# gnosisguild/pvw-rs

Measured on AMD Instinct MI355X. Metric: parties/s for n-party encrypt (pvw::crypto::encrypt); achieved HBM GB/s vs peak, higher is better.
Workload: dtype u64

## Files before the change

pvw_rs_amd/csrc/pvw_capi.hip:

```cpp
#include <hip/hip_runtime.h>

#include <algorithm>
#include <atomic>
#include <chrono>
#include <cmath>
#include <cstdio>
#include <cstring>
#include <functional>
#include <map>
#include <mutex>
#include <string>
#include <thread>
#include <vector>

#include "../../include/pvw_hip.h"
#include "pvw_arith.h"
#include "pvw_bignum.h"
#include "pvw_chacha.h"
#include "pvw_decode.h"
#include "pvw_kernels.h"
#include "pvw_shamir_fields.h"
#if PVW_TUNING
#include "../../include/pvw_hip_tuning.h"
#endif
// ... 107 lines not shown
  u64* gtmpB = nullptr;
  u64* gtmpK = nullptr;
  u64* shares = nullptr;
  size_t shares_bytes = 0;
  u64* interp = nullptr;
  size_t interp_bytes = 0;
  u64* interp_wide = nullptr;
  size_t interp_wide_bytes = 0;
  u64* packw = nullptr;
  size_t packw_bytes = 0;
  u64* packw_wide = nullptr;
  size_t packw_wide_bytes = 0;
  u64* handover_wide = nullptr;
  size_t handover_wide_bytes = 0;
  u64* handover_io = nullptr;
  size_t handover_io_bytes = 0;
  u64* correct = nullptr;
  size_t correct_bytes = 0;
  u64* correct_wide = nullptr;
  size_t correct_wide_bytes = 0;
  hipStream_t aux = nullptr;
  bool aux_used = false;
  std::vector<hipEvent_t> events;
  AheadRing ahead;
  char* ahead_block = nullptr;
  size_t ahead_set_bytes = 0, ahead_rhat_bytes = 0;
  std::vector<hipEvent_t> ahead_done;
  hipEvent_t ahead_guard[2] = {nullptr, nullptr};
  hipEvent_t ahead_mark = nullptr;
  hipEvent_t ahead_last = nullptr;
  bool ahead_off = false;
  struct Span { void* p; size_t bytes; bool cleared; };
  std::vector<Span> secrets, wiped;
  size_t rhat_public_from = SIZE_MAX;
};
static void ws_mark_secret(Workspace* w, void* p, size_t bytes, bool cleared = false) {
  if (!p || !bytes) return;
  if (p == (void*)w->rhat && w->rhat_public_from < bytes) w->rhat_public_from = bytes;
  for (Workspace::Span& sp : w->secrets)
    if (sp.p == p) { sp.bytes = bytes > sp.bytes ? bytes : sp.bytes; sp.cleared = cleared; return; }
  w->secrets.push_back(Workspace::Span{p, bytes, cleared});
}
static void ws_public(Workspace* w, void* p, size_t bytes) {
  if (!p || !bytes) return;
  const char *lo = (const char*)p, *hi = lo + bytes;
  for (const Workspace::Span& sp : w->secrets)
// ... 403 lines not shown
  hipFree(w->gtmpA);
  hipFree(w->gtmpB);
  hipFree(w->gtmpK);
  if (w->shares) hipMemset(w->shares, 0, w->shares_bytes);
  hipFree(w->shares);
  hipFree(w->interp);
  hipFree(w->interp_wide);
  hipFree(w->packw);
  hipFree(w->packw_wide);
  hipFree(w->handover_wide);
  if (w->handover_io) hipMemset(w->handover_io, 0, w->handover_io_bytes);
  hipFree(w->handover_io);
  if (w->correct) hipMemset(w->correct, 0, w->correct_bytes);
  hipFree(w->correct);
  if (w->correct_wide) hipMemset(w->correct_wide, 0, w->correct_wide_bytes);
  hipFree(w->correct_wide);
  for (hipEvent_t e : w->events) hipEventDestroy(e);
  if (w->ahead_block) hipMemset(w->ahead_block, 0, w->ahead_set_bytes * w->ahead.slots());
  hipFree(w->ahead_block);
  for (hipEvent_t e : w->ahead_done) hipEventDestroy(e);
  for (hipEvent_t e : w->ahead_guard) if (e) hipEventDestroy(e);
  if (w->ahead_mark) hipEventDestroy(w->ahead_mark);
  if (w->aux) hipStreamDestroy(w->aux);
  if (w->own_stream && w->stream) hipStreamDestroy(w->stream);
  delete w;
}
static int32_t ws_acquire(pvw_ctx* c, Workspace** out) {
  {
    std::lock_guard<std::mutex> g(c->mu);
    if (!c->pool.empty()) {
      *out = c->pool.back();
      c->pool.pop_back();
      return PVW_OK;
    }
  }
  Workspace* w = new Workspace();
  if (hipStreamCreateWithFlags(&w->stream, hipStreamNonBlocking) != hipSuccess) {
    delete w;
    return fail(PVW_ERR_INTERNAL, "hipStreamCreate failed");
  }
  w->own_stream = true;
  int32_t rc = ws_alloc(c, w);
  if (rc != PVW_OK) { ws_free(w); return rc; }
  *out = w;
  return PVW_OK;
}
// ... 115 lines not shown
  DealerKeys piece(size_t i) const { return by_state ? *this : from(i); }
  template <class Batch>
  void fill(Batch& b, u32 count) const {
    if (by_state) {
      b.rnd = st->dev;
      b.rnd_off = first;
    } else {
      for (u32 x = 0; x < count; ++x) b.key[x] = make_key(seeds + (first + x) * 32);
    }
  }
};

static int32_t ws_aux(Workspace* w, size_t events) {
  if (!w->aux) PVW_HIP(hipStreamCreateWithFlags(&w->aux, hipStreamNonBlocking));
  while (w->events.size() < events) {
    hipEvent_t e;
    PVW_HIP(hipEventCreateWithFlags(&e, hipEventDisableTiming));
    w->events.push_back(e);
  }
  w->aux_used = true;
  return PVW_OK;
}

template <class Body>
static int32_t host_call(pvw_ctx* c, Body&& body) {
  Workspace* w;
  PVW_TRY(ws_acquire(c, &w));
  int32_t rc = body(w);
  auto keep = [&](hipError_t e, const char* what) {
    if (e != hipSuccess && rc == PVW_OK) rc = fail(PVW_ERR_INTERNAL, std::string(what) + " failed: " + hipGetErrorString(e));
  };
  if (w->aux_used) keep(hipStreamSynchronize(w->aux), "helper stream sync");
  w->aux_used = false;
  keep(ws_wipe_secrets(w, w->stream), "wipe");
  keep(hipStreamSynchronize(w->stream), "stream sync");
  ws_release(c, w);
  return rc;
}

static bool multi_uses_gemm(size_t D) {
  const int gemm_min = (int)PVW_ENV_INT("PVW_GEMM_MIN_DEALERS", 3);
  return gemm_min > 0 && D >= (size_t)gemm_min;
}
static int32_t multi_capture_check(pvw_ctx* c, hipStream_t s, size_t D) {
  if (!multi_uses_gemm(D) || !stream_capturing(s)) return PVW_OK;
  bool ready;
  {
    std::lock_guard<std::mutex> g(c->init_mu);
    ready = c->xm_valid;
  }
  {
    std::lock_guard<std::mutex> g(c->mu);
    auto it = c->async_ws.find((void*)s);
    const Workspace* w = it == c->async_ws.end() ? nullptr : it->second;
    ready = ready && w && w->vhat16 && w->yd && w->sy && (w->gtmpA || !c->rowsA()) && (w->gtmpB || !c->rowsB());
  }
// ... 6 lines not shown
static int32_t deal_capture_check(pvw_ctx* c, hipStream_t s, size_t D) {
  if (!stream_capturing(s)) return PVW_OK;
  bool ready;
  {
    std::lock_guard<std::mutex> g(c->mu);
    auto it = c->async_ws.find((void*)s);
    ready = it != c->async_ws.end() && it->second->shares;
  }
  if (!ready)
    return fail(PVW_ERR_INVALID_PARAMETERS, "multi-dealer encrypt under stream capture: call pvw_prepare(PVW_PREPARE_MFMA) on "
                                            "this stream first (and again after the matrices change)");
  return multi_capture_check(c, s, D);
}

static hipStream_t call_stream(const pvw_ctx* c, void* stream) { return stream ? (hipStream_t)stream : c->stream; }
static int32_t sum_prepare(pvw_ctx* c, Workspace* w, hipStream_t s);
static int32_t device_ws(pvw_ctx* c, void* stream, hipStream_t* s, Workspace** w) {
  *s = call_stream(c, stream);
  return ws_for_stream(c, *s, w);
}
static int32_t device_end(Workspace* w, hipStream_t s, int32_t rc) {
  if (rc != PVW_OK) {
    if (w->aux) (void)hipStreamSynchronize(w->aux);
    (void)hipStreamSynchronize(s);
  }
  if (ws_wipe_secrets(w, s) != hipSuccess && rc == PVW_OK) rc = fail(PVW_ERR_INTERNAL, "wipe failed");
  return rc;
}

template <class Pre, class Body>
static int32_t device_call(pvw_ctx* c, void* stream, Pre&& pre, Body&& body) {
  PVW_TRY(ensure_device(c));
  const hipStream_t s = call_stream(c, stream);
  PVW_TRY(pre(s));
  Workspace* w;
  PVW_TRY(ws_for_stream(c, s, &w));
  return device_end(w, s, body(w, s));
}
template <class Body>
static int32_t device_call(pvw_ctx* c, void* stream, Body&& body) {
  return device_call(c, stream, [](hipStream_t) { return (int32_t)PVW_OK; }, body);
}

static int32_t validate_params(const pvw_params_t* p) {
  if (!p) return fail(PVW_ERR_INVALID_PARAMETERS, "params is NULL");
  if (p->n == 0) return fail(PVW_ERR_INVALID_PARAMETERS, "n must be > 0");
// ... 2457 lines not shown
        ProfScope ps(c, "vec_digits", s);
        PVW_HIP(launch_vec_digits(vh, (size_t)k * P, w->yd, w->sy, nv, k, L, l, c->dt, s, 0, 0, c->xm_bytes));
      }
      ProfScope ps(c, "gemm_digits", s);
      GemmSection a{c->xmA, c1g, c1g, w->gtmpA, rA, 0, 0}, b{c->xmB, c2g, c2g, w->gtmpB, rB, 0, 0};
      std::vector<GemmErrSource> es;
      if (fused_e2) {
        for (u32 v0 = 0; v0 < nv; v0 += PVW_MAX_PROLOGUE_KEYS) {
          GemmErrSource e{};
          e.span = (nv - v0) < PVW_MAX_PROLOGUE_KEYS ? (nv - v0) : PVW_MAX_PROLOGUE_KEYS;
          keys.from(d0 + v0).fill(e, e.span);
          e.key_v = 1;
          e.domain = DOM_E2; e.index0 = c->party_lo; e.index_row = 1; e.index_v = 0; e.bound = c->b2;
          e.scalars = gsc + c->party_lo; e.scalar_v = c->n;
          es.push_back(e);
        }
        b.addend = nullptr;
      }
      if (rs && last) {
        GemmSection& fin = rB ? b : a;
        fin.rnd_ctr = &rs->counter;
        fin.rnd_adv = D;
      }
      PVW_HIP(launch_gemm_digits(a, b, w->yd, w->sy, c->dt, k, L, l, nv, (size_t)rA * P, (size_t)rB * P, s, nullptr, fused_e2 ? es.data() : nullptr, c->xm_bytes));
    } else {
      ProfScope ps(c, "mac_rows_multi", s);
      MacSection a(c->dA, c1g, c1g, rA), b(c->dB, c2g, c2g, rB);
      MultiVec mv{vh, (size_t)k * P, (size_t)rA * P, (size_t)rB * P, nv};
      if (rs && last) {
        a.rnd_ctr = &rs->counter;
        a.rnd_adv = D;
      }
      PVW_HIP(launch_mac_rows_multi(a, b, mv, c->dt, k, L, l, s));
    }
  }
  if (out_repr == PVW_REPR_POWER) {
    ProfScope ps(c, "intt", s);
    PVW_HIP(launch_ntt(d_c1, D * rA, true, c->dt, L, l, s));
    PVW_HIP(launch_ntt(d_c2, D * rB, true, c->dt, L, l, s));
  }
  return PVW_OK;
}

static int32_t encrypt_multi_checks(pvw_ctx* c, size_t D, size_t per_dealer, uint32_t out_repr) {
  PVW_TRY(check_repr(out_repr));
  if (D == 0) return fail(PVW_ERR_INVALID_PARAMETERS, "no dealers");
  if (per_dealer != c->n) {
// ... 3572 lines not shown
    PVW_TRY(cbd_job(c->variance, sj));
    draw.key = make_key(ks.sk_seed); draw.cbd_half = sj.cbd_half; draw.cbd_v = sj.cbd_v;
  } else {
    PVW_TRY(ws_aux(w, 2 * (size_t)nchunks + 2));
  }
  auto upload = [&](u32 ci, hipStream_t st) -> int32_t {
    const u32 q0 = a + ci * chunk, cn = (b - q0) < chunk ? (b - q0) : chunk;
    const size_t wd = (size_t)cn * k * l;
    i64* dst = d_small2[ci & 1];
    PVW_HIP(hipMemcpyAsync(dst, sk + (size_t)(q0 - lo) * k * l, wd * 8, hipMemcpyHostToDevice, st));
    if (ek) PVW_HIP(hipMemcpyAsync(dst + (size_t)chunk * k * l, ek + (size_t)(q0 - lo) * k * l, wd * 8, hipMemcpyHostToDevice, st));
    return PVW_OK;
  };
  if (!ks.seeded()) PVW_TRY(upload(0, s));
  PVW_HIP(launch_untile(c->dA, d_api, k, 0, k, L, l, false, c->dt, s));
  PVW_HIP(launch_vec_digits(d_api, P, d_yd, d_sy, k, k, L, l, c->dt, s, l, (size_t)k * P));
  for (u32 ci = 0; ci < nchunks; ++ci) {
    const u32 p0 = a + ci * chunk;
    const u32 cnt = (b - p0) < chunk ? (b - p0) : chunk;
    i64* d_small = d_small2[ci & 1];
    if (ci > 0 && !ks.seeded()) PVW_HIP(hipStreamWaitEvent(s, w->events[2 * ci], 0));
    ProfScope ps(c, "keygen", s);
    GemmSection ga{d_xm, d_erow, d_erow, d_tmp, cnt, 0, 0}, gb{nullptr, nullptr, nullptr, nullptr, 0, 0, 0};
    ga.tiled_out = c->dB;
    ga.tiled_row0 = p0 - c->party_lo;
    ga.tiled_swap = 1;
    ga.row_stride = (size_t)k * P;
    if (direct) {
      draw.party0 = p0;
      PVW_HIP(launch_shat_mftile(ks.seeded() ? nullptr : d_small, ks.seeded() ? &draw : nullptr, d_xm, cnt, k, L, l, c->dt, s));
      GemmErrSource es{};
      if (ek) { es.explicit_coeffs = d_small + (size_t)chunk * k * l; es.coef_row = k; es.coef_v = 1; }
      else es.key[0] = make_key(seed);
      es.domain = DOM_EKEY; es.index0 = p0 * k; es.index_row = k; es.index_v = 1; es.bound = c->b1;
      ga.addend = nullptr;
      ga.out = nullptr;
      PVW_HIP(launch_gemm_digits(ga, gb, d_yd, d_sy, c->dt, k, L, l, k, P, 0, s, &es));
    } else {
      PrologueBatch pb{};
      if (seed) pb.key[0] = make_key(seed);
      PrologueJob& js = pb.job[0];
      PrologueJob& je = pb.job[1];
      PVW_TRY(ks.job(c, pb, js, d_small, p0));
      js.out = d_srow; js.stride_poly = P; js.stride_limb = l; js.rep_out = (size_t)k * P;
      je.sj.kind = SAMPLE_UNIFORM; je.sj.domain = DOM_EKEY; je.sj.index0 = p0 * k; je.sj.count = k; je.sj.bound = c->b1;
      je.rep_index0 = k;
      if (ek) { je.explicit_coeffs = d_small + (size_t)chunk * k * l; je.rep_coeffs = (size_t)k * l; }
      je.out = d_erow; je.stride_poly = P; je.stride_limb = l; je.rep_out = (size_t)k * P;
      pb.njobs = 2;
      pb.reps = cnt;
      PVW_HIP(launch_prologue(pb, c->dt, L, l, s));
      PVW_HIP(hipMemsetAsync(d_xm, 0, xm_words(cnt, k, L, l) * 8, s));
      PVW_HIP(launch_mftile(d_srow, false, d_xm, cnt, k, L, l, s));
      PVW_HIP(launch_gemm_digits(ga, gb, d_yd, d_sy, c->dt, k, L, l, k, P, 0, s));
    }
    if (ks.seeded()) continue;
    PVW_HIP(hipEventRecord(w->events[2 * ci + 1], s));
    if (ci + 1 < nchunks) {
      if (ci >= 1) PVW_HIP(hipStreamWaitEvent(w->aux, w->events[2 * (ci - 1) + 1], 0));
      PVW_TRY(upload(ci + 1, w->aux));
      PVW_HIP(hipEventRecord(w->events[2 * ci + 2], w->aux));
    }
  }
  return PVW_OK;
}

static int32_t keygen_transposed(pvw_ctx* c, Workspace* w, u32 a, u32 b, u32 lo, const KeySource& ks, const int64_t* ek,
                                 const uint8_t* seed, bool use_gemm) {
  const u32 k = c->k, l = c->l, L = c->L;
  const size_t P = c->poly();
  hipStream_t s = w->stream;
  const u32 group = use_gemm ? 16 : 4;
  u32 sg = group;
  if (use_gemm) {
    const size_t per16 = yd_bytes(16, k, L, l);
    size_t m = ((size_t)2 << 30) / (per16 ? per16 : 1);
    if (m < 1) m = 1;
// ... 527 lines not shown
```

pvw_rs_amd/csrc/pvw_gemm.hip:

```cpp
#include <hip/hip_runtime.h>

#include "pvw_arith.h"
#include "pvw_chacha.h"
#include "pvw_decode.h"
#include "pvw_kernels.h"
#include "pvw_dev.h"

namespace pvw {

__global__ __launch_bounds__(64) void mfma_i8_probe_kernel(const signed char* __restrict__ A,
                                                            const signed char* __restrict__ B, int* __restrict__ Cm) {
  const u32 l = threadIdx.x, r = l & 31, h = l >> 5;
  union { v4i32 v; signed char b[16]; } fa, fb;
#pragma unroll
  for (int j = 0; j < 16; ++j) {
    fa.b[j] = A[r * 32 + 16 * h + j];
    fb.b[j] = B[(16 * h + j) * 32 + r];
  }
  v16i32 acc = {};
  acc = __builtin_amdgcn_mfma_i32_32x32x32_i8(fa.v, fb.v, acc, 0, 0, 0);
#pragma unroll
  for (int g = 0; g < 16; ++g) Cm[((g & 3) + 8 * (g >> 2) + 4 * h) * 32 + r] = acc[g];
}

// ... 661 lines not shown
  for (int r = 0; r < 2; ++r) {
    const u32 rt = rtbase + 2 * wr + r;
    if (rt >= RT || rt * 32 >= sec.nrows) continue;
    const u32 row = rt * 32 + rr;
#pragma unroll
    for (int g = 0; g < 4; ++g) {
      u64 res[2];
      if (biased) gemm_recombine_biased<FASTQ>(acc[r][g], m, inv32, res);
      else gemm_recombine<FASTQ>(acc[r][g], m, inv32, res);
#pragma unroll
      for (int pr = 0; pr < 2; ++pr) {
        const u32 v = g * 4 + pr + 2 * h;
        if (row < sec.nrows && v < nv)
          sec.tmp[vb * sec.tmp_bstride + (((size_t)limb * ELL + slot) * nv_pad + v) * rows_pad + row] = res[pr];
      }
    }
  }
}

#define PVW_FINISH_VPB (ELL >= 64 ? 2 : 4)
template <int ELL>
__global__ __launch_bounds__(256) void gemm_finish_kernel(GemmSection sec, const Mod* __restrict__ mods, u32 L,
                                                           u32 nv, u32 nv_pad, u32 rows_pad, size_t ostride,
                                                           const int* __restrict__ SY, size_t sy_b16) {
  constexpr int VPB = PVW_FINISH_VPB, PT = 32 * ELL / 256 ? 32 * ELL / 256 : 1;
  static_assert(sizeof(u64) * VPB * ELL * 33 <= 48 * 1024 || ELL > 32, "finish tiles");
  __shared__ u64 tile[VPB][ELL][33];
  rnd_advance(sec.rnd_ctr, sec.rnd_adv);
  const u32 rb = blockIdx.x, v0 = blockIdx.y * VPB, limb = blockIdx.z;
  const u32 row0 = rb * 32;
  u64 in[VPB][PT];
#pragma unroll
  for (int vi = 0; vi < VPB; ++vi) {
    const u32 v = (v0 + vi) < nv ? (v0 + vi) : (nv - 1);
    const u64* tp = sec.tmp + (v >> 4) * sec.tmp_bstride + (((size_t)limb * ELL) * nv_pad + (nv_pad == 16 ? (v & 15) : v)) * rows_pad + row0;
#pragma unroll
    for (int x = 0; x < PT; ++x) {
      const u32 e = threadIdx.x + 256 * x;
      const u32 row = e & 31, slot = (e >> 5) % ELL;
      in[vi][x] = tp[(size_t)slot * nv_pad * rows_pad + row];
    }
  }
#pragma unroll
  for (int vi = 0; vi < VPB; ++vi)
#pragma unroll
    for (int x = 0; x < PT; ++x) {
      const u32 e = threadIdx.x + 256 * x;
      if (e < 32 * ELL) tile[vi][(e >> 5) % ELL][e & 31] = in[vi][x];
    }
  __syncthreads();
  const u64 q = mods[limb].q;
  u64 add[VPB][PT];
// ... 18 lines not shown
#pragma unroll
    for (int x = 0; x < PT; ++x) {
      const u32 e = threadIdx.x + 256 * x;
      const u32 slot = e % ELL, row = e / ELL;
      if (e < 32 * ELL && row0 + row < sec.nrows && v0 + vi < nv) {
        const u64 val = addmod(tile[vi][slot][row], add[vi][x], q);
        if (sec.tiled_out) {
          constexpr u32 R = 128 / ELL;
          const u32 prow = sec.tiled_row0 + (sec.tiled_swap ? row0 + row : v0 + vi);
          const u32 pcol = sec.tiled_swap ? v0 + vi : row0 + row;
          const u32 ncol = sec.tiled_swap ? nv : sec.nrows;
          sec.tiled_out[(((size_t)(prow / R) * L + limb) * ncol + pcol) * 128 + (prow % R) * ELL + slot] = val;
        } else {
          const size_t o = (size_t)(v0 + vi) * ostride + (size_t)(row0 + row) * rstride + (size_t)limb * ELL + slot;
          sec.out[o] = val;
        }
      }
    }
}

template <int ELL, int VPB>
__global__ __launch_bounds__(32 * VPB) void gemm_finish_err_kernel(GemmSection sec, DevTables t, u32 L, u32 nv, u32 nv_pad, u32 rows_pad,
                                                               size_t ostride, const int* __restrict__ SY, size_t sy_b16, GemmErrSource es,
                                                               u32 v_lo, u32 v_hi) {
  constexpr int G = ELL / 2;
  constexpr int CST = ELL + 2;
  __shared__ i64 coef[32 * VPB * CST];
  const u32 tid = threadIdx.x, lane = tid & 63;
  const u32 row_raw = blockIdx.x * 32 + (tid & 31), v_raw = v_lo + blockIdx.y * VPB + (tid >> 5);
  const bool v_ok = v_raw < v_hi;
  const u32 row = row_raw < sec.nrows ? row_raw : sec.nrows - 1, v = v_ok ? v_raw : v_hi - 1;
  rnd_advance(sec.rnd_ctr, sec.rnd_adv);
  i64 c[ELL];
  __shared__ ChaChaKey vkey[VPB];
  if (es.rnd && !es.explicit_coeffs) {
    if ((tid & 31) == 0) vkey[tid >> 5] = call_seed(es.rnd->seed, es.rnd->base + es.rnd_off + (u64)(v - v_lo) * es.key_v);
    __builtin_amdgcn_fence(__ATOMIC_RELEASE, "wavefront");
    __builtin_amdgcn_wave_barrier();
    __builtin_amdgcn_fence(__ATOMIC_ACQUIRE, "wavefront");
  }
  {
    i64* o = coef + tid * CST;
    if (es.explicit_coeffs) {
      const i64* ec = es.explicit_coeffs + ((size_t)row * es.coef_row + (size_t)v * es.coef_v) * ELL;
#pragma unroll
      for (int sl = 0; sl < ELL; sl += 2) *reinterpret_cast<v2u64*>(o + sl) = *reinterpret_cast<const v2u64*>(ec + sl);
    } else {
      ChaChaRng g;
      g.init(es.rnd ? vkey[tid >> 5] : es.key[(v - v_lo) * es.key_v], es.domain, es.index0 + row * es.index_row + v * es.index_v);
      auto emit = [o](u32 sl, i64 val) { o[sl] = val; };
      sample_uniform_poly(g, ELL, es.bound, emit);
    }
#pragma unroll
    for (int sl = 0; sl < ELL; ++sl) c[sl] = o[sl];
  }
  const i64 scalar = es.scalars ? (i64)es.scalars[(size_t)v * es.scalar_v + row] : 0;
  const u64* tbase = sec.tmp + (v >> 4) * sec.tmp_bstride + (size_t)(nv_pad == 16 ? (v & 15) : v) * rows_pad + row;
  const size_t sstride = (size_t)nv_pad * rows_pad;
  const u64* cbase = reinterpret_cast<const u64*>(SY + (size_t)(v >> 4) * sy_b16 + ((size_t)((v & 15) >> 2) * L * ELL) * 32) + (v & 3);
  constexpr u32 R = 128 / ELL;
  const size_t rstride = sec.row_stride ? sec.row_stride : (size_t)L * ELL;
  u64 in[ELL];
  auto load_tmp = [&](u32 limb) {
#pragma unroll
    for (int sl = 0; sl < ELL; ++sl) in[sl] = __builtin_nontemporal_load(tbase + ((size_t)limb * ELL + sl) * sstride);
  };
  const u32 per = (L + gridDim.z - 1) / gridDim.z, limb_end = (blockIdx.z + 1) * per < L ? (blockIdx.z + 1) * per : L;
  u32 limb = blockIdx.z * per;
  if (limb < limb_end) load_tmp(limb);
  u64* stg = reinterpret_cast<u64*>(coef) + (size_t)(tid - lane) * CST;
  const u32 gi = lane & (G - 1), gb = lane & ~(u32)(G - 1);
  for (; limb < limb_end; ++limb) {
    const Mod m = t.mods[limb];
    u64 a[ELL], x[ELL];
#pragma unroll
    for (int sl = 0; sl < ELL; ++sl) { a[sl] = signed_residue(c[sl], m); x[sl] = in[sl]; }
    if (limb + 1 < limb_end) load_tmp(limb + 1);
    ntt_forward<ELL>(a, t.tw + (size_t)limb * ELL, t.twp + (size_t)limb * ELL, m);
    if (es.scalars) {
      const u64 mr = signed_residue(scalar, m);
      const u64* g = t.ghat + (size_t)limb * ELL;
      const u64* gp = t.ghatp + (size_t)limb * ELL;
#pragma unroll
      for (int sl = 0; sl < ELL; ++sl) a[sl] = addmod(a[sl], mulmod_shoup(mr, g[sl], gp[sl], m.q), m.q);
    }
#pragma unroll
    for (int sl = 0; sl < ELL; sl += 2) {
      const u64 c0 = cbase[((size_t)limb * ELL + sl) * 16], c1 = cbase[((size_t)limb * ELL + sl + 1) * 16];
      *reinterpret_cast<v2u64*>(stg + lane * CST + sl) =
          (v2u64){addmod(addmod(x[sl], a[sl], m.q), c0, m.q), addmod(addmod(x[sl + 1], a[sl + 1], m.q), c1, m.q)};
    }
// ... 71 lines not shown
  if (nv % 4) {
    const u32 NVG = (nv + 3) / 4, JB = gemm_ktiles(k, bytes);
    hipError_t e = hipMemsetAsync(YD + (size_t)(NVG - 1) * L * ell * JB * 1024, 0, (size_t)L * ell * JB * 1024, s);
    if (e != hipSuccess) return e;
    e = hipMemsetAsync(SY + (size_t)(NVG - 1) * L * ell * 32, 0, (size_t)L * ell * 32 * sizeof(int), s);
    if (e != hipSuccess) return e;
  }
  if (bytes == 7) {
    PVW_DISPATCH_ELL(ell, vec_digits7_kernel<E><<<dim3(nv * L * ell), dim3(64), 0, s>>>(vhat, vstride, YD, SY, nv, k, L, t, lstride, jstride));
    return hipGetLastError();
  }
#if PVW_TUNING
  static const int stage = (int)PVW_ENV_INT("PVW_VEC_DIGITS_STAGE", 1);
  if (!stage) {
    PVW_DISPATCH_ELL(ell, vec_digits_kernel<E, false><<<dim3(nv * L * ell), dim3(64), 0, s>>>(vhat, vstride, YD, SY, nv, k, L, t, lstride, jstride));
    return hipGetLastError();
  }
#endif
  PVW_DISPATCH_ELL(ell, vec_digits_kernel<E, true><<<dim3(nv * L * ell), dim3(64), 0, s>>>(vhat, vstride, YD, SY, nv, k, L, t, lstride, jstride));
  return hipGetLastError();
}

hipError_t launch_gemm_digits_core(GemmSection& sa, GemmSection& sb, const signed char* YD, const int* SY,
                                   const DevTables& t, u32 k, u32 L, u32 ell, u32 nv, hipStream_t s, u32 bytes) {
  const u32 kt = gemm_ktiles(k, bytes);
  sa.rt_groups = (sa.nrows + PVW_GEMM_ROWS_PER_WG - 1) / PVW_GEMM_ROWS_PER_WG;
  sb.rt_groups = (sb.nrows + PVW_GEMM_ROWS_PER_WG - 1) / PVW_GEMM_ROWS_PER_WG;
  const u32 blocks = (sa.rt_groups + sb.rt_groups) * L * ell;
  if (blocks == 0 || nv == 0) return hipSuccess;
  const u32 vbn = (nv + 15) / 16;
  const u32 NVG = vbn > 1 ? 4 : (nv + 3) / 4;
  const u32 nv_pad = NVG * 4;
  sa.tmp_bstride = (size_t)L * ell * 16 * sa.rt_groups * PVW_GEMM_ROWS_PER_WG;
  sb.tmp_bstride = (size_t)L * ell * 16 * sb.rt_groups * PVW_GEMM_ROWS_PER_WG;
  const size_t yd_b16 = (size_t)4 * L * ell * kt * 1024, sy_b16 = sy_bytes(16, L, ell) / sizeof(int);
#define PVW_GEMM_LAUNCH(G, N)                                                                                              \
  do {                                                                                                                    \
    if (t.min_q_bits >= 55) { PVW_DISPATCH_ELL(ell, gemm_digits_kernel<E, G, PVW_GEMM_RPW, N, true><<<dim3(blocks * vbn), dim3(256), 0, s>>>(sa, sb, YD, SY, t.mods, k, L, nv, nv_pad, vbn, yd_b16, sy_b16, kt)); } \
    else { PVW_DISPATCH_ELL(ell, gemm_digits_kernel<E, G, PVW_GEMM_RPW, N, false><<<dim3(blocks * vbn), dim3(256), 0, s>>>(sa, sb, YD, SY, t.mods, k, L, nv, nv_pad, vbn, yd_b16, sy_b16, kt)); } \
  } while (0)
#if PVW_TUNING
  if (PVW_ENV_INT("PVW_GEMM_ZERO_OPERANDS", 0)) {
    if (sa.nrows) (void)hipMemsetAsync(const_cast<u64*>(sa.XM), 0, xm_words(sa.nrows, k, L, ell) * 8, s);
    if (sb.nrows) (void)hipMemsetAsync(const_cast<u64*>(sb.XM), 0, xm_words(sb.nrows, k, L, ell) * 8, s);
    (void)hipMemsetAsync(const_cast<signed char*>(YD), 0, yd_b16 * vbn, s);
  }
#endif
  const bool wide = vbn >= 2 && k % 16 == 0 && k >= 16 && kt % 2 == 0 && PVW_ENV_INT("PVW_GEMM_WIDE", 1) != 0;
  if (wide) {
    const u32 ga = (sa.rt_groups * 4 + 7) / 8, gb2 = (sb.rt_groups * 4 + 7) / 8;
    const u32 wblocks = (ga + gb2) * L * ell * ((vbn + 1) / 2);
    if (t.min_q_bits >= 55) { PVW_DISPATCH_ELL(ell, gemm_digits_wide_kernel<E, true><<<dim3(wblocks), dim3(512), 0, s>>>(sa, sb, YD, t.mods, k, L, nv, nv_pad, vbn, yd_b16, kt)); }
    else { PVW_DISPATCH_ELL(ell, gemm_digits_wide_kernel<E, false><<<dim3(wblocks), dim3(512), 0, s>>>(sa, sb, YD, t.mods, k, L, nv, nv_pad, vbn, yd_b16, kt)); }
  } else {
  static const int unroll_ok = (int)PVW_ENV_INT("PVW_GEMM_UNROLL", 1);
  if (NVG == 4 && unroll_ok && kt == 64) { PVW_GEMM_LAUNCH(4, 8); }
  else if (NVG == 4 && unroll_ok && kt == 128) { PVW_GEMM_LAUNCH(4, 16); }
  else switch (NVG) {
    case 1: PVW_GEMM_LAUNCH(1, 0); break;
    case 2: PVW_GEMM_LAUNCH(2, 0); break;
    case 3: PVW_GEMM_LAUNCH(3, 0); break;
    case 4: PVW_GEMM_LAUNCH(4, 0); break;
    default: return hipErrorInvalidValue;
  }
#undef PVW_GEMM_LAUNCH
  }
  return hipGetLastError();
}

hipError_t launch_gemm_digits(const GemmSection& a, const GemmSection& b, const signed char* YD, const int* SY,
                              const DevTables& t, u32 k, u32 L, u32 ell, u32 nv, size_t ostride_a, size_t ostride_b,
                              hipStream_t s, const GemmErrSource* es_a, const GemmErrSource* es_b, u32 bytes) {
  GemmSection sa = a, sb = b;
  if ((sa.nrows == 0 && sb.nrows == 0) || nv == 0) return hipSuccess;
  {
    const hipError_t ge = launch_gemm_digits_core(sa, sb, YD, SY, t, k, L, ell, nv, s, bytes);
    if (ge != hipSuccess) return ge;
  }
  const u32 vbn = (nv + 15) / 16;
  const u32 nv_pad = (vbn > 1 ? 4 : (nv + 3) / 4) * 4;
  const size_t sy_b16 = sy_bytes(16, L, ell) / sizeof(int);
  auto finish = [&](const GemmSection& sec, size_t ostride, const GemmErrSource* es) -> hipError_t {
    if (!sec.nrows) return hipSuccess;
    const u32 rows_pad = sec.rt_groups * PVW_GEMM_ROWS_PER_WG;
    if (es) {
      if (ell > 32 || (sec.tiled_out && !sec.tiled_swap) || (!sec.tiled_out && !sec.out)) return hipErrorInvalidValue;
      for (u32 v_lo = 0; v_lo < nv; ++es) {
        const u32 span = es->span && es->span < nv - v_lo ? es->span : nv - v_lo, v_hi = v_lo + span;
        GemmSection sec_l = sec;
        if (v_hi < nv) sec_l.rnd_ctr = nullptr;
        const u32 gx = (sec.nrows + 31) / 32;
        bool one_wave = false;
#if PVW_TUNING
        one_wave = PVW_ENV_INT("PVW_FINISH_VPB", 8) == 2;
        if (one_wave) {
          const dim3 grid(gx, (span + 1) / 2, 1);
          switch (ell) {
            case 8: gemm_finish_err_kernel<8, 2><<<grid, dim3(64), 0, s>>>(sec_l, t, L, nv, nv_pad, rows_pad, ostride, SY, sy_b16, *es, v_lo, v_hi); break;
            case 16: gemm_finish_err_kernel<16, 2><<<grid, dim3(64), 0, s>>>(sec_l, t, L, nv, nv_pad, rows_pad, ostride, SY, sy_b16, *es, v_lo, v_hi); break;
            default: gemm_finish_err_kernel<32, 2><<<grid, dim3(64), 0, s>>>(sec_l, t, L, nv, nv_pad, rows_pad, ostride, SY, sy_b16, *es, v_lo, v_hi); break;
          }
        }
#endif
        if (!one_wave) {
          const u32 gy = (span + 7) / 8;
          u32 lz = 1;
          const size_t want = (size_t)PVW_ENV_INT("PVW_FINISH_BLOCKS", 4096);
          while (lz < L && (size_t)gx * gy * lz < want) lz *= 2;
          if (lz > L) lz = L;
          const dim3 grid(gx, gy, lz);
          switch (ell) {
            case 8: gemm_finish_err_kernel<8, 8><<<grid, dim3(256), 0, s>>>(sec_l, t, L, nv, nv_pad, rows_pad, ostride, SY, sy_b16, *es, v_lo, v_hi); break;
            case 16: gemm_finish_err_kernel<16, 8><<<grid, dim3(256), 0, s>>>(sec_l, t, L, nv, nv_pad, rows_pad, ostride, SY, sy_b16, *es, v_lo, v_hi); break;
            default: gemm_finish_err_kernel<32, 8><<<grid, dim3(256), 0, s>>>(sec_l, t, L, nv, nv_pad, rows_pad, ostride, SY, sy_b16, *es, v_lo, v_hi); break;
          }
        }
        v_lo = v_hi;
      }
      return hipGetLastError();
    }
    PVW_DISPATCH_ELL(ell, gemm_finish_kernel<E><<<dim3((sec.nrows + 31) / 32, (nv + (E >= 64 ? 2 : 4) - 1) / (E >= 64 ? 2 : 4), L), dim3(256), 0, s>>>(
                              sec, t.mods, L, nv, nv_pad, rows_pad, ostride, SY, sy_b16));
    return hipGetLastError();
  };
  hipError_t fe = finish(sa, ostride_a, es_a);
  if (fe != hipSuccess) return fe;
  return finish(sb, ostride_b, es_b);
}
static inline u32 ilog2_u32(u32 x) { u32 b = 0; while ((1u << b) < x) ++b; return b; }

__global__ __launch_bounds__(256) void gemm_finish_decrypt_kernel(const u64* __restrict__ tmp, size_t tmp_bstride, u32 nv_pad,
                                                                  u32 rows_pad, const int* __restrict__ SY, size_t sy_b16,
                                                                  const Mod* __restrict__ mods, u32 ell_log2, u32 P, u32 nrows,
                                                                  u32 nv, const u64* __restrict__ c2, size_t c2_vstride,
                                                                  size_t c2_rstride, u64* __restrict__ noisy) {
  constexpr u32 TR = 128, TF = 32;
  __shared__ __attribute__((aligned(16))) u64 tile[TR][TF + 2];
  const u32 r0 = blockIdx.x * TR, f0 = blockIdx.y * TF, v = blockIdx.z;
  const u32 wave = threadIdx.x >> 6, lane = threadIdx.x & 63;
  const u64* tb = tmp + (size_t)(v >> 4) * tmp_bstride + (size_t)(v & 15) * rows_pad + r0 + 2 * lane;
  const size_t fstride = (size_t)nv_pad * rows_pad;
  const u64* cb = reinterpret_cast<const u64*>(SY + (size_t)(v >> 4) * sy_b16 + (size_t)((v & 15) >> 2) * P * 32) + (v & 3);
  v2u64 x[TF / 4];
#pragma unroll
  for (u32 i = 0; i < TF / 4; ++i) {
    const u32 f = f0 + wave + 4 * i;
    if (f < P) x[i] = __builtin_nontemporal_load(reinterpret_cast<const v2u64*>(tb + (size_t)f * fstride));
  }
#pragma unroll
  for (u32 i = 0; i < TF / 4; ++i) {
// ... 58 lines not shown
```

pvw_rs_amd/csrc/pvw_kernels.h:

```cpp
#pragma once
#include <hip/hip_runtime.h>

#include "pvw_arith.h"
#include "pvw_chacha.h"
#include "pvw_decode.h"
#include "pvw_wide.h"

#ifndef PVW_TUNING
#define PVW_TUNING 0
#endif
#if PVW_TUNING
#include <cstdlib>
#define PVW_ENV_INT(name, dflt) ([]() -> long { const char* e_ = getenv(name); return e_ ? atol(e_) : (long)(dflt); }())
#else
#define PVW_ENV_INT(name, dflt) ((long)(dflt))
#endif

namespace pvw {

enum { DOM_R = 0, DOM_E1 = 1, DOM_E2 = 2, DOM_SK = 3, DOM_EKEY = 4, DOM_CRS = 5, DOM_GAUSS = 6, DOM_PK = 7, DOM_CALL = 8 };

struct RndState {
  u32 seed[8];
  u64 counter;
// ... 427 lines not shown
                         const Mod* mods = nullptr);
struct ShatDraw {
  ChaChaKey key;
  u32 cbd_half, cbd_v;
  u32 party0;
};
hipError_t launch_shat_mftile(const i64* coeffs, const ShatDraw* draw, u64* XM, u32 rows, u32 k, u32 L, u32 ell, const DevTables& t,
                              hipStream_t s);
hipError_t launch_vec_digits(const u64* vhat, size_t vstride, signed char* YD, int* SY, u32 nv, u32 k, u32 L, u32 ell,
                             const DevTables& t, hipStream_t s, size_t lstride = 0, size_t jstride = 0, u32 bytes = 8);
struct GemmErrSource {
  u32 span;
  const i64* explicit_coeffs;
  size_t coef_row, coef_v;
  ChaChaKey key[PVW_MAX_PROLOGUE_KEYS];
  u32 key_v;
  u32 domain, index0, index_row, index_v;
  u64 bound;
  const u64* scalars;
  size_t scalar_v;
  const RndState* rnd;
  u64 rnd_off;
};
hipError_t launch_gemm_digits(const GemmSection& a, const GemmSection& b, const signed char* YD, const int* SY,
                              const DevTables& t, u32 k, u32 L, u32 ell, u32 nv, size_t ostride_a, size_t ostride_b,
                              hipStream_t s, const GemmErrSource* es_a = nullptr, const GemmErrSource* es_b = nullptr, u32 bytes = 8);
hipError_t launch_gemm_digits_core(GemmSection& a, GemmSection& b, const signed char* YD, const int* SY, const DevTables& t, u32 k,
                                   u32 L, u32 ell, u32 nv, hipStream_t s, u32 bytes = 8);
hipError_t launch_finish_decrypt(const GemmSection& a, const int* SY, const DevTables& t, u32 L, u32 ell, u32 nv, const u64* c2,
                                 size_t c2_vstride, size_t c2_rstride, u64* noisy, hipStream_t s);
hipError_t launch_reduce_words(const u64* src, u64* dst, size_t words, const DevTables& t, u32 L, u32 ell, hipStream_t s);
#if PVW_TUNING
hipError_t read_stamps(u64* out, u32* hw, u32 count);
hipError_t init_probe_attributes();
hipError_t launch_read_probe(const u64* M, size_t total_tiles, u32 tiles_per_wave, u64* sink, hipStream_t s);
hipError_t launch_read_probe2(const u64* M, size_t total_tiles, u32 tiles_per_wave, u64* sink, u32 U, bool dbuf, u32 lds_bytes,
                              hipStream_t s, u32 xmap = 0);
#endif
hipError_t init_kernel_attributes();
hipError_t launch_mfma_probe(const signed char* A, const signed char* B, int* C, hipStream_t s);
hipError_t launch_decode(u64* noisy, u64* out, size_t count, const DecodeTables& t, hipStream_t s, const DevTables* xf = nullptr,
                         u64* wipe = nullptr, size_t wipe_bytes = 0, bool* wiped = nullptr, u64* noise = nullptr,
                         u32* status = nullptr, const PlainArgs* plain = nullptr);

hipError_t launch_wire_pack(const u64* words, size_t count, unsigned char* out, const Mod* mods, u32 L, u32 ell, hipStream_t s);
hipError_t launch_wire_unpack(const unsigned char* in, size_t count, u64* words, unsigned long long* bad, const Mod* mods, u32 L,
                              u32 ell, hipStream_t s);
hipError_t init_wire_attributes();

}
```

Baseline: 22.47 million.

## Split GEMM by limb ranges and overlap finish kernels on a side stream

Partitions the multi-dealer GEMM and its finish step into limb ranges (two by default). Each range's GEMM runs on the main stream while the previous range's finish or error-injection kernel runs on a dedicated side stream, joined by events. The goal is to hide finish-kernel time behind GEMM work. The cost is extra launches, event traffic and a second stream, and it is disabled under stream capture.

```diff
diff --git a/pvw_rs_amd/csrc/pvw_capi.hip b/pvw_rs_amd/csrc/pvw_capi.hip
--- a/pvw_rs_amd/csrc/pvw_capi.hip
+++ b/pvw_rs_amd/csrc/pvw_capi.hip
@@ -153,6 +153,10 @@
   hipStream_t aux = nullptr;
   bool aux_used = false;
   std::vector<hipEvent_t> events;
+  hipStream_t fin = nullptr;
+  bool fin_used = false;
+  bool fin_off = false;
+  hipEvent_t fin_ev[GemmRanges::MAX + 1] = {};
   AheadRing ahead;
   char* ahead_block = nullptr;
   size_t ahead_set_bytes = 0, ahead_rhat_bytes = 0;
@@ -602,6 +606,8 @@
   for (hipEvent_t e : w->ahead_guard) if (e) hipEventDestroy(e);
   if (w->ahead_mark) hipEventDestroy(w->ahead_mark);
   if (w->aux) hipStreamDestroy(w->aux);
+  for (hipEvent_t e : w->fin_ev) if (e) hipEventDestroy(e);
+  if (w->fin) hipStreamDestroy(w->fin);
   if (w->own_stream && w->stream) hipStreamDestroy(w->stream);
   delete w;
 }
@@ -763,6 +769,32 @@
   return PVW_OK;
 }
 
+#define PVW_GEMM_FINISH_RANGES_ENCRYPT 2
+#define PVW_GEMM_FINISH_RANGES_KEYGEN 2
+static const GemmRanges* ws_gemm_ranges(Workspace* w, hipStream_t s, u32 measured, GemmRanges& gr) {
+  long z = PVW_ENV_INT("PVW_GEMM_FINISH_RANGES", 0);
+  if (z <= 0) z = measured;
+  if (z > GemmRanges::MAX) z = GemmRanges::MAX;
+  if (z <= 1 || w->fin_off || stream_capturing(s)) return nullptr;
+  if (!w->fin) {
+    bool ok = hipStreamCreateWithFlags(&w->fin, hipStreamNonBlocking) == hipSuccess;
+    for (hipEvent_t& e : w->fin_ev) ok = ok && hipEventCreateWithFlags(&e, hipEventDisableTiming) == hipSuccess;
+    if (!ok) {
+      (void)hipGetLastError();
+      for (hipEvent_t& e : w->fin_ev) { if (e) hipEventDestroy(e); e = nullptr; }
+      if (w->fin) hipStreamDestroy(w->fin);
+      w->fin = nullptr;
+      w->fin_off = true;
+      return nullptr;
+    }
+  }
+  w->fin_used = true;
+  gr.side = w->fin;
+  gr.ev = w->fin_ev;
+  gr.ranges = (u32)z;
+  return &gr;
+}
+
 template <class Body>
 static int32_t host_call(pvw_ctx* c, Body&& body) {
   Workspace* w;
@@ -773,6 +805,8 @@
   };
   if (w->aux_used) keep(hipStreamSynchronize(w->aux), "helper stream sync");
   w->aux_used = false;
+  if (w->fin_used) keep(hipStreamSynchronize(w->fin), "finish stream sync");
+  w->fin_used = false;
   keep(ws_wipe_secrets(w, w->stream), "wipe");
   keep(hipStreamSynchronize(w->stream), "stream sync");
   ws_release(c, w);
@@ -825,6 +859,7 @@
 static int32_t device_end(Workspace* w, hipStream_t s, int32_t rc) {
   if (rc != PVW_OK) {
     if (w->aux) (void)hipStreamSynchronize(w->aux);
+    if (w->fin) (void)hipStreamSynchronize(w->fin);
     (void)hipStreamSynchronize(s);
   }
   if (ws_wipe_secrets(w, s) != hipSuccess && rc == PVW_OK) rc = fail(PVW_ERR_INTERNAL, "wipe failed");
@@ -3328,7 +3363,9 @@
         fin.rnd_ctr = &rs->counter;
         fin.rnd_adv = D;
       }
-      PVW_HIP(launch_gemm_digits(a, b, w->yd, w->sy, c->dt, k, L, l, nv, (size_t)rA * P, (size_t)rB * P, s, nullptr, fused_e2 ? es.data() : nullptr, c->xm_bytes));
+      GemmRanges gr;
+      PVW_HIP(launch_gemm_digits(a, b, w->yd, w->sy, c->dt, k, L, l, nv, (size_t)rA * P, (size_t)rB * P, s, nullptr, fused_e2 ? es.data() : nullptr, c->xm_bytes,
+                                 ws_gemm_ranges(w, s, PVW_GEMM_FINISH_RANGES_ENCRYPT, gr)));
     } else {
       ProfScope ps(c, "mac_rows_multi", s);
       MacSection a(c->dA, c1g, c1g, rA), b(c->dB, c2g, c2g, rB);
@@ -6947,6 +6984,7 @@
     if (ci > 0 && !ks.seeded()) PVW_HIP(hipStreamWaitEvent(s, w->events[2 * ci], 0));
     ProfScope ps(c, "keygen", s);
     GemmSection ga{d_xm, d_erow, d_erow, d_tmp, cnt, 0, 0}, gb{nullptr, nullptr, nullptr, nullptr, 0, 0, 0};
+    GemmRanges gr;
     ga.tiled_out = c->dB;
     ga.tiled_row0 = p0 - c->party_lo;
     ga.tiled_swap = 1;
@@ -6960,7 +6998,7 @@
       es.domain = DOM_EKEY; es.index0 = p0 * k; es.index_row = k; es.index_v = 1; es.bound = c->b1;
       ga.addend = nullptr;
       ga.out = nullptr;
-      PVW_HIP(launch_gemm_digits(ga, gb, d_yd, d_sy, c->dt, k, L, l, k, P, 0, s, &es));
+      PVW_HIP(launch_gemm_digits(ga, gb, d_yd, d_sy, c->dt, k, L, l, k, P, 0, s, &es, nullptr, 8, ws_gemm_ranges(w, s, PVW_GEMM_FINISH_RANGES_KEYGEN, gr)));
     } else {
       PrologueBatch pb{};
       if (seed) pb.key[0] = make_key(seed);
@@ -6977,7 +7015,7 @@
       PVW_HIP(launch_prologue(pb, c->dt, L, l, s));
       PVW_HIP(hipMemsetAsync(d_xm, 0, xm_words(cnt, k, L, l) * 8, s));
       PVW_HIP(launch_mftile(d_srow, false, d_xm, cnt, k, L, l, s));
-      PVW_HIP(launch_gemm_digits(ga, gb, d_yd, d_sy, c->dt, k, L, l, k, P, 0, s));
+      PVW_HIP(launch_gemm_digits(ga, gb, d_yd, d_sy, c->dt, k, L, l, k, P, 0, s, nullptr, nullptr, 8, ws_gemm_ranges(w, s, PVW_GEMM_FINISH_RANGES_KEYGEN, gr)));
     }
     if (ks.seeded()) continue;
     PVW_HIP(hipEventRecord(w->events[2 * ci + 1], s));
diff --git a/pvw_rs_amd/csrc/pvw_gemm.hip b/pvw_rs_amd/csrc/pvw_gemm.hip
--- a/pvw_rs_amd/csrc/pvw_gemm.hip
+++ b/pvw_rs_amd/csrc/pvw_gemm.hip
@@ -707,12 +707,12 @@
 template <int ELL>
 __global__ __launch_bounds__(256) void gemm_finish_kernel(GemmSection sec, const Mod* __restrict__ mods, u32 L,
                                                            u32 nv, u32 nv_pad, u32 rows_pad, size_t ostride,
-                                                           const int* __restrict__ SY, size_t sy_b16) {
+                                                           const int* __restrict__ SY, size_t sy_b16, u32 limb0) {
   constexpr int VPB = PVW_FINISH_VPB, PT = 32 * ELL / 256 ? 32 * ELL / 256 : 1;
   static_assert(sizeof(u64) * VPB * ELL * 33 <= 48 * 1024 || ELL > 32, "finish tiles");
   __shared__ u64 tile[VPB][ELL][33];
   rnd_advance(sec.rnd_ctr, sec.rnd_adv);
-  const u32 rb = blockIdx.x, v0 = blockIdx.y * VPB, limb = blockIdx.z;
+  const u32 rb = blockIdx.x, v0 = blockIdx.y * VPB, limb = limb0 + blockIdx.z;
   const u32 row0 = rb * 32;
   u64 in[VPB][PT];
 #pragma unroll
@@ -777,7 +777,7 @@
 template <int ELL, int VPB>
 __global__ __launch_bounds__(32 * VPB) void gemm_finish_err_kernel(GemmSection sec, DevTables t, u32 L, u32 nv, u32 nv_pad, u32 rows_pad,
                                                                size_t ostride, const int* __restrict__ SY, size_t sy_b16, GemmErrSource es,
-                                                               u32 v_lo, u32 v_hi) {
+                                                               u32 v_lo, u32 v_hi, u32 limb0, u32 nl) {
   constexpr int G = ELL / 2;
   constexpr int CST = ELL + 2;
   __shared__ i64 coef[32 * VPB * CST];
@@ -820,8 +820,8 @@
 #pragma unroll
     for (int sl = 0; sl < ELL; ++sl) in[sl] = __builtin_nontemporal_load(tbase + ((size_t)limb * ELL + sl) * sstride);
   };
-  const u32 per = (L + gridDim.z - 1) / gridDim.z, limb_end = (blockIdx.z + 1) * per < L ? (blockIdx.z + 1) * per : L;
-  u32 limb = blockIdx.z * per;
+  const u32 per = (nl + gridDim.z - 1) / gridDim.z, limb_end = limb0 + ((blockIdx.z + 1) * per < nl ? (blockIdx.z + 1) * per : nl);
+  u32 limb = limb0 + blockIdx.z * per;
   if (limb < limb_end) load_tmp(limb);
   u64* stg = reinterpret_cast<u64*>(coef) + (size_t)(tid - lane) * CST;
   const u32 gi = lane & (G - 1), gb = lane & ~(u32)(G - 1);
@@ -939,11 +939,14 @@
 }
 
 hipError_t launch_gemm_digits_core(GemmSection& sa, GemmSection& sb, const signed char* YD, const int* SY,
-                                   const DevTables& t, u32 k, u32 L, u32 ell, u32 nv, hipStream_t s, u32 bytes) {
+                                   const DevTables& t, u32 k, u32 L, u32 ell, u32 nv, hipStream_t s, u32 bytes, u32 limb0,
+                                   u32 nl) {
   const u32 kt = gemm_ktiles(k, bytes);
   sa.rt_groups = (sa.nrows + PVW_GEMM_ROWS_PER_WG - 1) / PVW_GEMM_ROWS_PER_WG;
   sb.rt_groups = (sb.nrows + PVW_GEMM_ROWS_PER_WG - 1) / PVW_GEMM_ROWS_PER_WG;
-  const u32 blocks = (sa.rt_groups + sb.rt_groups) * L * ell;
+  if (nl == 0) { limb0 = 0; nl = L; }
+  if (limb0 + nl > L) return hipErrorInvalidValue;
+  const u32 blocks = (sa.rt_groups + sb.rt_groups) * nl * ell;
   if (blocks == 0 || nv == 0) return hipSuccess;
   const u32 vbn = (nv + 15) / 16;
   const u32 NVG = vbn > 1 ? 4 : (nv + 3) / 4;
@@ -951,10 +954,19 @@
   sa.tmp_bstride = (size_t)L * ell * 16 * sa.rt_groups * PVW_GEMM_ROWS_PER_WG;
   sb.tmp_bstride = (size_t)L * ell * 16 * sb.rt_groups * PVW_GEMM_ROWS_PER_WG;
   const size_t yd_b16 = (size_t)4 * L * ell * kt * 1024, sy_b16 = sy_bytes(16, L, ell) / sizeof(int);
+  GemmSection ka = sa, kb = sb;
+  const size_t ls0 = (size_t)limb0 * ell;
+  for (GemmSection* ks : {&ka, &kb}) {
+    if (!ks->nrows) continue;
+    ks->XM += ls0 * (ks->rt_groups * 4 * PVW_GEMM_RPW) * kt * 128;
+    ks->tmp += ls0 * nv_pad * ks->rt_groups * PVW_GEMM_ROWS_PER_WG;
+  }
+  const signed char* yd0 = YD + ls0 * kt * 1024;
+  const Mod* mods = t.mods + limb0;
 #define PVW_GEMM_LAUNCH(G, N)                                                                                              \
   do {                                                                                                                    \
-    if (t.min_q_bits >= 55) { PVW_DISPATCH_ELL(ell, gemm_digits_kernel<E, G, PVW_GEMM_RPW, N, true><<<dim3(blocks * vbn), dim3(256), 0, s>>>(sa, sb, YD, SY, t.mods, k, L, nv, nv_pad, vbn, yd_b16, sy_b16, kt)); } \
-    else { PVW_DISPATCH_ELL(ell, gemm_digits_kernel<E, G, PVW_GEMM_RPW, N, false><<<dim3(blocks * vbn), dim3(256), 0, s>>>(sa, sb, YD, SY, t.mods, k, L, nv, nv_pad, vbn, yd_b16, sy_b16, kt)); } \
+    if (t.min_q_bits >= 55) { PVW_DISPATCH_ELL(ell, gemm_digits_kernel<E, G, PVW_GEMM_RPW, N, true><<<dim3(blocks * vbn), dim3(256), 0, s>>>(ka, kb, yd0, SY, mods, k, L, nv, nv_pad, vbn, yd_b16, sy_b16, kt)); } \
+    else { PVW_DISPATCH_ELL(ell, gemm_digits_kernel<E, G, PVW_GEMM_RPW, N, false><<<dim3(blocks * vbn), dim3(256), 0, s>>>(ka, kb, yd0, SY, mods, k, L, nv, nv_pad, vbn, yd_b16, sy_b16, kt)); } \
   } while (0)
 #if PVW_TUNING
   if (PVW_ENV_INT("PVW_GEMM_ZERO_OPERANDS", 0)) {
@@ -966,9 +978,9 @@
   const bool wide = vbn >= 2 && k % 16 == 0 && k >= 16 && kt % 2 == 0 && PVW_ENV_INT("PVW_GEMM_WIDE", 1) != 0;
   if (wide) {
     const u32 ga = (sa.rt_groups * 4 + 7) / 8, gb2 = (sb.rt_groups * 4 + 7) / 8;
-    const u32 wblocks = (ga + gb2) * L * ell * ((vbn + 1) / 2);
-    if (t.min_q_bits >= 55) { PVW_DISPATCH_ELL(ell, gemm_digits_wide_kernel<E, true><<<dim3(wblocks), dim3(512), 0, s>>>(sa, sb, YD, t.mods, k, L, nv, nv_pad, vbn, yd_b16, kt)); }
-    else { PVW_DISPATCH_ELL(ell, gemm_digits_wide_kernel<E, false><<<dim3(wblocks), dim3(512), 0, s>>>(sa, sb, YD, t.mods, k, L, nv, nv_pad, vbn, yd_b16, kt)); }
+    const u32 wblocks = (ga + gb2) * nl * ell * ((vbn + 1) / 2);
+    if (t.min_q_bits >= 55) { PVW_DISPATCH_ELL(ell, gemm_digits_wide_kernel<E, true><<<dim3(wblocks), dim3(512), 0, s>>>(ka, kb, yd0, mods, k, L, nv, nv_pad, vbn, yd_b16, kt)); }
+    else { PVW_DISPATCH_ELL(ell, gemm_digits_wide_kernel<E, false><<<dim3(wblocks), dim3(512), 0, s>>>(ka, kb, yd0, mods, k, L, nv, nv_pad, vbn, yd_b16, kt)); }
   } else {
   static const int unroll_ok = (int)PVW_ENV_INT("PVW_GEMM_UNROLL", 1);
   if (NVG == 4 && unroll_ok && kt == 64) { PVW_GEMM_LAUNCH(4, 8); }
@@ -987,18 +999,21 @@
 
 hipError_t launch_gemm_digits(const GemmSection& a, const GemmSection& b, const signed char* YD, const int* SY,
                               const DevTables& t, u32 k, u32 L, u32 ell, u32 nv, size_t ostride_a, size_t ostride_b,
-                              hipStream_t s, const GemmErrSource* es_a, const GemmErrSource* es_b, u32 bytes) {
+                              hipStream_t s, const GemmErrSource* es_a, const GemmErrSource* es_b, u32 bytes,
+                              const GemmRanges* gr) {
   GemmSection sa = a, sb = b;
   if ((sa.nrows == 0 && sb.nrows == 0) || nv == 0) return hipSuccess;
-  {
-    const hipError_t ge = launch_gemm_digits_core(sa, sb, YD, SY, t, k, L, ell, nv, s, bytes);
-    if (ge != hipSuccess) return ge;
-  }
   const u32 vbn = (nv + 15) / 16;
+  u32 Z = gr && gr->side && gr->ev && vbn >= 2 ? gr->ranges : 1;
+  if (Z > GemmRanges::MAX) Z = GemmRanges::MAX;
+  if (Z > (L + 1) / 2) Z = (L + 1) / 2;
+  if (Z < 1) Z = 1;
   const u32 nv_pad = (vbn > 1 ? 4 : (nv + 3) / 4) * 4;
   const size_t sy_b16 = sy_bytes(16, L, ell) / sizeof(int);
-  auto finish = [&](const GemmSection& sec, size_t ostride, const GemmErrSource* es) -> hipError_t {
-    if (!sec.nrows) return hipSuccess;
+  auto finish = [&](const GemmSection& sec_in, size_t ostride, const GemmErrSource* es, hipStream_t fs, u32 l0, u32 nl, bool adv) -> hipError_t {
+    if (!sec_in.nrows) return hipSuccess;
+    GemmSection sec = sec_in;
+    if (!adv) sec.rnd_ctr = nullptr;
     const u32 rows_pad = sec.rt_groups * PVW_GEMM_ROWS_PER_WG;
     if (es) {
       if (ell > 32 || (sec.tiled_out && !sec.tiled_swap) || (!sec.tiled_out && !sec.out)) return hipErrorInvalidValue;
@@ -1013,9 +1028,9 @@
         if (one_wave) {
           const dim3 grid(gx, (span + 1) / 2, 1);
           switch (ell) {
-            case 8: gemm_finish_err_kernel<8, 2><<<grid, dim3(64), 0, s>>>(sec_l, t, L, nv, nv_pad, rows_pad, ostride, SY, sy_b16, *es, v_lo, v_hi); break;
-            case 16: gemm_finish_err_kernel<16, 2><<<grid, dim3(64), 0, s>>>(sec_l, t, L, nv, nv_pad, rows_pad, ostride, SY, sy_b16, *es, v_lo, v_hi); break;
-            default: gemm_finish_err_kernel<32, 2><<<grid, dim3(64), 0, s>>>(sec_l, t, L, nv, nv_pad, rows_pad, ostride, SY, sy_b16, *es, v_lo, v_hi); break;
+            case 8: gemm_finish_err_kernel<8, 2><<<grid, dim3(64), 0, fs>>>(sec_l, t, L, nv, nv_pad, rows_pad, ostride, SY, sy_b16, *es, v_lo, v_hi, l0, nl); break;
+            case 16: gemm_finish_err_kernel<16, 2><<<grid, dim3(64), 0, fs>>>(sec_l, t, L, nv, nv_pad, rows_pad, ostride, SY, sy_b16, *es, v_lo, v_hi, l0, nl); break;
+            default: gemm_finish_err_kernel<32, 2><<<grid, dim3(64), 0, fs>>>(sec_l, t, L, nv, nv_pad, rows_pad, ostride, SY, sy_b16, *es, v_lo, v_hi, l0, nl); break;
           }
         }
 #endif
@@ -1023,26 +1038,45 @@
           const u32 gy = (span + 7) / 8;
           u32 lz = 1;
           const size_t want = (size_t)PVW_ENV_INT("PVW_FINISH_BLOCKS", 4096);
-          while (lz < L && (size_t)gx * gy * lz < want) lz *= 2;
-          if (lz > L) lz = L;
+          while (lz < nl && (size_t)gx * gy * lz < want) lz *= 2;
+          if (lz > nl) lz = nl;
           const dim3 grid(gx, gy, lz);
           switch (ell) {
-            case 8: gemm_finish_err_kernel<8, 8><<<grid, dim3(256), 0, s>>>(sec_l, t, L, nv, nv_pad, rows_pad, ostride, SY, sy_b16, *es, v_lo, v_hi); break;
-            case 16: gemm_finish_err_kernel<16, 8><<<grid, dim3(256), 0, s>>>(sec_l, t, L, nv, nv_pad, rows_pad, ostride, SY, sy_b16, *es, v_lo, v_hi); break;
-            default: gemm_finish_err_kernel<32, 8><<<grid, dim3(256), 0, s>>>(sec_l, t, L, nv, nv_pad, rows_pad, ostride, SY, sy_b16, *es, v_lo, v_hi); break;
+            case 8: gemm_finish_err_kernel<8, 8><<<grid, dim3(256), 0, fs>>>(sec_l, t, L, nv, nv_pad, rows_pad, ostride, SY, sy_b16, *es, v_lo, v_hi, l0, nl); break;
+            case 16: gemm_finish_err_kernel<16, 8><<<grid, dim3(256), 0, fs>>>(sec_l, t, L, nv, nv_pad, rows_pad, ostride, SY, sy_b16, *es, v_lo, v_hi, l0, nl); break;
+            default: gemm_finish_err_kernel<32, 8><<<grid, dim3(256), 0, fs>>>(sec_l, t, L, nv, nv_pad, rows_pad, ostride, SY, sy_b16, *es, v_lo, v_hi, l0, nl); break;
           }
         }
         v_lo = v_hi;
       }
       return hipGetLastError();
     }
-    PVW_DISPATCH_ELL(ell, gemm_finish_kernel<E><<<dim3((sec.nrows + 31) / 32, (nv + (E >= 64 ? 2 : 4) - 1) / (E >= 64 ? 2 : 4), L), dim3(256), 0, s>>>(
-                              sec, t.mods, L, nv, nv_pad, rows_pad, ostride, SY, sy_b16));
+    PVW_DISPATCH_ELL(ell, gemm_finish_kernel<E><<<dim3((sec.nrows + 31) / 32, (nv + (E >= 64 ? 2 : 4) - 1) / (E >= 64 ? 2 : 4), nl), dim3(256), 0, fs>>>(
+                              sec, t.mods, L, nv, nv_pad, rows_pad, ostride, SY, sy_b16, l0));
     return hipGetLastError();
   };
-  hipError_t fe = finish(sa, ostride_a, es_a);
-  if (fe != hipSuccess) return fe;
-  return finish(sb, ostride_b, es_b);
+  hipError_t rc = hipSuccess;
+  bool forked = false;
+  for (u32 z = 0, l0 = 0; z < Z && rc == hipSuccess; ++z) {
+    const u32 nl = L / Z + (z < L % Z ? 1 : 0);
+    hipStream_t fs = s;
+    rc = launch_gemm_digits_core(sa, sb, YD, SY, t, k, L, ell, nv, s, bytes, l0, nl);
+    if (rc == hipSuccess && Z > 1) {
+      fs = gr->side;
+      rc = hipEventRecord(gr->ev[z], s);
+      if (rc == hipSuccess) rc = hipStreamWaitEvent(fs, gr->ev[z], 0);
+      forked = forked || rc == hipSuccess;
+    }
+    if (rc == hipSuccess) rc = finish(sa, ostride_a, es_a, fs, l0, nl, z + 1 == Z);
+    if (rc == hipSuccess) rc = finish(sb, ostride_b, es_b, fs, l0, nl, z + 1 == Z);
+    l0 += nl;
+  }
+  if (forked) {
+    hipError_t je = hipEventRecord(gr->ev[Z], gr->side);
+    if (je == hipSuccess) je = hipStreamWaitEvent(s, gr->ev[Z], 0);
+    if (rc == hipSuccess) rc = je;
+  }
+  return rc;
 }
 static inline u32 ilog2_u32(u32 x) { u32 b = 0; while ((1u << b) < x) ++b; return b; }
 
diff --git a/pvw_rs_amd/csrc/pvw_kernels.h b/pvw_rs_amd/csrc/pvw_kernels.h
--- a/pvw_rs_amd/csrc/pvw_kernels.h
+++ b/pvw_rs_amd/csrc/pvw_kernels.h
@@ -473,11 +473,18 @@
   const RndState* rnd;
   u64 rnd_off;
 };
+struct GemmRanges {
+  enum { MAX = 4 };
+  hipStream_t side;
+  const hipEvent_t* ev;
+  u32 ranges;
+};
 hipError_t launch_gemm_digits(const GemmSection& a, const GemmSection& b, const signed char* YD, const int* SY,
                               const DevTables& t, u32 k, u32 L, u32 ell, u32 nv, size_t ostride_a, size_t ostride_b,
-                              hipStream_t s, const GemmErrSource* es_a = nullptr, const GemmErrSource* es_b = nullptr, u32 bytes = 8);
+                              hipStream_t s, const GemmErrSource* es_a = nullptr, const GemmErrSource* es_b = nullptr, u32 bytes = 8,
+                              const GemmRanges* gr = nullptr);
 hipError_t launch_gemm_digits_core(GemmSection& a, GemmSection& b, const signed char* YD, const int* SY, const DevTables& t, u32 k,
-                                   u32 L, u32 ell, u32 nv, hipStream_t s, u32 bytes = 8);
+                                   u32 L, u32 ell, u32 nv, hipStream_t s, u32 bytes = 8, u32 limb0 = 0, u32 nl = 0);
 hipError_t launch_finish_decrypt(const GemmSection& a, const int* SY, const DevTables& t, u32 L, u32 ell, u32 nv, const u64* c2,
                                  size_t c2_vstride, size_t c2_rstride, u64* noisy, hipStream_t s);
 hipError_t launch_reduce_words(const u64* src, u64* dst, size_t words, const DevTables& t, u32 L, u32 ell, hipStream_t s);
```

Result: no change. 22.41 million (-0.2%).
